# loicland/superpoint_graph

Hardware: AMD Instinct MI355X
Metric: superpoints/sec (embed+ECC fwd+bwd), S3DIS-shaped SPG (higher is better)
Workload: dtype f32; 1 GPU; gru_10_0,f_13 fwd+bwd+Adam; 1 scene/GPU x 1000 sp x 128 pts x 14 f, 5000 edges x 13 f; hipgraph=False, step_call=spg_train_step (one library call: forward + backward), parallelism=single GPU, batchnorm=per-rank statistics, precision=f32

## Files before the change

### include/spg_hip.h

```cpp
#ifndef SPG_HIP_H
#define SPG_HIP_H
#include <stddef.h>
#include <stdint.h>

#ifdef __cplusplus
extern "C" {
#endif

#define SPG_MAX_LAYERS 8
#define SPG_VERSION 200

const char* spg_last_error(void);
int spg_version(void);

size_t spg_graph_workspace_bytes(int N, int n_src, int E);
int spg_graph_build(const int64_t* idxn, const int64_t* degs, int N, int n_src, int E, void* graph_ws, void* stream);
int spg_graph_export(const void* graph_ws, int N, int n_src, int E, int32_t* rowptr, int32_t* src, int32_t* dst,
                     int32_t* rev_rowptr, int32_t* rev_eid, int32_t* hdr, void* stream);

int spg_ecc_aggregate_fwd(int dtype, const void* x, const void* w, const int64_t* idxe, const void* graph_ws, int N,
                          int E, int cin, int cout, int w_is_matrix, void* out, void* stream);
int spg_ecc_aggregate_bwd(int dtype, const void* x, const void* w, const int64_t* idxe, const void* graph_ws, int N,
                          int E, int n_x_rows, int n_w_rows, int cin, int cout, int w_is_matrix, const void* grad_out,
                          void* grad_x, void* grad_w, void* stream);
// ... 246 lines not shown
  float* desc;
  float* grad_desc;
  const spg_eccrnn_cfg* ecc_cfg;
  int E;
  const void* graph_ws;
  const float* edgefeats;
  const void* const* ecc_params;
  void* const* ecc_grads;
  void* ecc_ws; void* ecc_bwd_ws;
  float* ecc_out;
  float* grad_ecc_out;
  int nout, n_classes;
  const float* cls_W; const float* cls_b;
  float* cls_dW; float* cls_db;
  float* cls_work;
  float* logits;
  float* grad_logits;
  const int64_t* target;
  const float* class_weight;
  int64_t ignore_index;
  int reduction_mean;
  float* loss_buf;
  int ptn_slots_clean;
} spg_step_args;
int spg_train_step(const spg_step_args* args, void* stream);
int spg_infer_step(const spg_step_args* args, void* stream);
int spg_cross_entropy_fwd_bwd(const float* logits, const int64_t* target, const float* weight, int N, int C, int64_t ignore_index,
                              int reduction_mean, float* loss, float* lse, float* wsum, float* grad_logits, void* stream);

int spg_ecc_persistent_errors(void);
int spg_ecc_persistent_errors_clear(void);
int spg_ecc_persistent_status(int* errors, int* withheld, int clear);
int spg_prof_read_tag(int tag, double* ms, long* launches, double* flops);

int spg_group_trace(void* buf, int max_launches);
int spg_group_trace_read(int* out, int max);

#define SPG_TILES_VERTICES_PER_BLOCK 32
int spg_neighbourhood_tiles(const float* xyz, const float* rgb, long N, const void* nei, int nei_is_i64, long K, int k, const int64_t* rows,
                            long m, int cloud_rgb, const float* elevation, const float* xyn, int own_rgb, int own_xy, int flags,
                            float* clouds, float* clouds_global, float* diameters, int32_t* error_flag, void* stream);
int spg_augment_whole(const float* xyz, const float* rgb, long N, const float* M, const float* ref_point, const float* noise_xyz,
                      const float* noise_rgb, float* xyz_out, float* rgb_out, void* stream);
size_t spg_random_subgraph_workspace_bytes(long n);
int spg_random_subgraph(const int32_t* rowptr, const uint32_t* inc, const int32_t* ends, long E, long n, int subgraph_size,
                        const int64_t* seeds, int n_seeds, uint8_t* selected_ver, uint8_t* selected_edg, int64_t* state, void* workspace,
                        size_t workspace_bytes, void* stream);
size_t spg_induced_subgraph_workspace_bytes(long n, long E);
int spg_induced_subgraph(const int32_t* ends, long E, long n, const uint8_t* selected_ver, const uint8_t* selected_edg, int64_t* rows,
                         int64_t* new_ver_index, int64_t* kept_edges, int64_t* edg_source, int64_t* edg_target, int64_t* counts,
                         void* workspace, size_t workspace_bytes, void* stream);

enum { SPG_STRUCTURE_IDS_NONE = 0, SPG_STRUCTURE_IDS_OBJECTS = 1, SPG_STRUCTURE_IDS_LABELS = 2, SPG_STRUCTURE_IDS_GIVEN = 3 };
size_t spg_structure_frame_workspace_bytes(long n);
int spg_structure_frame(const float* xyz, long n, float* frame, int32_t* error_flag, void* workspace, size_t workspace_bytes, void* stream);
int spg_structure_vertices(const float* xyz, long n, const float* frame, const uint8_t* rgb_u8, const void* hist, int hist_cols,
                           int id_mode, const void* ids_in, int ids_is_i64, float* elevation, float* xyn, float* rgb, float* geof,
                           int64_t* hard_ids, void* stream);
int spg_structure_edges(const int32_t* knn_idx, long n, int k_local, int k_adj, const int64_t* hard_ids, int64_t* edg_source,
                        int64_t* edg_target, uint8_t* is_transition, uint8_t* active, int32_t* error_flag, void* stream);

size_t spg_plane_workspace_bytes(long n, long n_low, int trials);
int spg_plane_low(const float* xyz, long n, float low_height, int32_t* low_index, int32_t* n_low, int32_t* error_flag, void* workspace,
                  size_t workspace_bytes, void* stream);
int spg_plane_fit(const float* xyz, long n, const int32_t* low_index, long n_low, const int32_t* subsets, int trials, float* elevation,
                  double* coef, double* intercept, float* threshold, uint8_t* inlier_mask, int32_t* result, int32_t* error_flag,
// ... 22 lines not shown
```

### superpoint_graph_amd/_lib.py

```python
from __future__ import annotations

import ctypes
import os
import subprocess

import torch

_HERE = os.path.dirname(os.path.abspath(__file__))
CSRC = os.path.join(_HERE, 'csrc')
LIB_PATH = os.environ.get('SPG_HIP_LIB') or os.path.join(CSRC, 'libspg_hip.so')

SPG_MAX_LAYERS = 8
SPG_MAX_PARTS = 64
c_void_pp = ctypes.POINTER(ctypes.c_void_p)


class PointNetCfg(ctypes.Structure):
    _fields_ = [('nfeat', ctypes.c_int), ('nfeat_stn', ctypes.c_int), ('nfeat_global', ctypes.c_int), ('npts', ctypes.c_int),
                ('n_stn_conv', ctypes.c_int), ('n_stn_fc', ctypes.c_int), ('n_conv', ctypes.c_int), ('n_fc', ctypes.c_int),
                ('stn_conv', ctypes.c_int * SPG_MAX_LAYERS), ('stn_fc', ctypes.c_int * SPG_MAX_LAYERS),
                ('conv', ctypes.c_int * SPG_MAX_LAYERS), ('fc', ctypes.c_int * SPG_MAX_LAYERS),
                ('last_ac', ctypes.c_int), ('bn_eps', ctypes.c_float), ('bn_momentum', ctypes.c_float)]


# ... 144 lines not shown
    'spg_structure_vertices': (_i, [_p, _l, _p, _p, _p, _i, _i, _p, _i, _p, _p, _p, _p, _p, _p]),
    'spg_structure_edges': (_i, [_p, _l, _i, _i, _p, _p, _p, _p, _p, _p, _p]),
    'spg_plane_workspace_bytes': (_sz, [_l, _l, _i]),
    'spg_plane_low': (_i, [_p, _l, ctypes.c_float, _p, _p, _p, _p, _sz, _p]),
    'spg_plane_fit': (_i, [_p, _l, _p, _l, _p, _i, _p, _p, _p, _p, _p, _p, _p, _p, _sz, _p]),
    'spg_parsed_workspace_bytes': (_sz, [_l]),
    'spg_parsed_stats': (_i, [_p, _l, _i, _p, _p, _p, _p, _p, _sz, _p]),
    'spg_parsed_rows': (_i, [_i, _p, _l, _p, _i, _p, _p, _i, _p, _p, _p, _p, _l, _p, _i, _p, _p, _l, _p, _p, _p]),
    'spg_class_count': (_i, [_p, _i, _l, _i, _p, _p]),
    'spg_sample_spg_workspace_bytes': (_sz, [_l, _l]),
    'spg_sample_spg': (_i, [_p, _l, _l, _p, _p, _l, _p, _p, _i, _i, _l, _l, _p, _p, _p, _p, _p, _p, _p, _sz, _p]),
    'spg_edge_features': (_i, [ctypes.POINTER(EdgeFeatureSpecs), _p, _l, _p, _p, _p, _p]),
    'spg_loader_random': (_i, [_p, _p, _p, _i, _i, _i, ctypes.c_uint64, ctypes.c_uint32, _i, ctypes.c_float, _i, ctypes.c_float, _i, _p, _p, _p, _p]),
    'spg_cross_entropy_fwd': (_i, [_p, _p, _p, _i, _i, ctypes.c_int64, _i, _p, _p, _p, _p]),
    'spg_cross_entropy_bwd': (_i, [_p, _p, _p, _p, _p, _p, _i, _i, ctypes.c_int64, _i, _p, _p]),
    'spg_cross_entropy_fwd_bwd': (_i, [_p, _p, _p, _i, _i, ctypes.c_int64, _i, _p, _p, _p, _p, _p]),
    'spg_train_step': (_i, [ctypes.POINTER(StepArgs), _p]),
    'spg_infer_step': (_i, [ctypes.POINTER(StepArgs), _p]),
    'spg_eval_accumulate': (_i, [_p, _i, _l, _i, _i, _p, _p, _p, _p, _p, _p]),
    'spg_set_bn_allreduce': (_i, [_p, _p, _p, _l]),
    'spg_rccl_unique_id': (_i, [_p]),
    'spg_rccl_init': (_i, [_p, _i, _i]),
    'spg_rccl_world_size': (_i, []),
    'spg_rccl_allreduce_sum_f32': (_i, [_p, _l, _p]),
    'spg_rccl_sync_bn': (_i, [_p, _l]),
    'spg_rccl_sync_slots': (_i, [_i]),
    'spg_group_trace': (_i, [_p, _i]),
    'spg_group_trace_read': (_i, [_p, _i]),
    'spg_rccl_allreduce_sum_f64': (_i, [_p, _l, _p]),
    'spg_set_slot_allreduce': (_i, [_p, _p, _i]),
    'spg_rccl_destroy': (_i, []),
    'spg_prof_enable': (None, [_i]),
    'spg_prof_tag': (_i, [_i, _i, _i, _i, _i, _i]),
    'spg_prof_read_tag': (_i, [_i, ctypes.POINTER(ctypes.c_double), ctypes.POINTER(ctypes.c_long), ctypes.POINTER(ctypes.c_double)]),
    'spg_prof_read_shapes': (_i, [ctypes.POINTER(_i), ctypes.POINTER(ctypes.c_double), _i]),
    'spg_tune': (_i, [_i, _i]),
    'spg_prof_read': (_i, [ctypes.POINTER(ctypes.c_double), ctypes.POINTER(ctypes.c_long), ctypes.POINTER(ctypes.c_double), _i]),
}

_lib = None


def build(verbose: bool = False) -> str:
    out = subprocess.run(['make', '-C', CSRC, '-j8'], capture_output=True, text=True)
    if out.returncode != 0:
        raise RuntimeError('building libspg_hip.so failed:\n' + out.stdout[-4000:] + out.stderr[-4000:])
    if verbose:
        print(out.stdout[-2000:])
    return LIB_PATH


def lib():
    global _lib
    if _lib is None:
        if not os.path.exists(LIB_PATH):
            raise RuntimeError(f'{LIB_PATH} not found: the HIP extension is not built '
                               f'(run `python -c "import __graft_entry__ as g; g.build()"` or `make -C {CSRC}`). '
                               'There is no CPU fallback for the product path.')
        L = ctypes.CDLL(LIB_PATH)
        for name, (res, args) in SIGNATURES.items():
            fn = getattr(L, name)
            fn.restype = res
            fn.argtypes = args
        _lib = L
    return _lib

# ... 6 lines not shown
```

### superpoint_graph_amd/csrc/spg_common.h

```cpp
#pragma once
#include <float.h>
#include <hip/hip_runtime.h>
#include <stdint.h>
#include <stdio.h>
#include <string.h>

typedef float f32x16 __attribute__((ext_vector_type(16)));
typedef float f32x4 __attribute__((ext_vector_type(4)));

#define SPG_KC 32
#define SPG_MAX_DEVICES 16
#define SPG_THREADS 256

extern "C" const char* spg_last_error(void);
void spg_set_error(const char* fmt, ...);
enum { SPG_TUNE_NO_PERSIST = 0, SPG_TUNE_DBG = 3, SPG_TUNE_FIN_SLICE_MIN = 4, SPG_TUNE_NO_STAT_ACCUM = 5, SPG_TUNE_NO_HEAD_SERVICE = 6, SPG_TUNE_PRECISION = 7,
       SPG_TUNE_NO_PERSIST_ECC = 8, SPG_TUNE_NO_BN_FOLD = 10, SPG_TUNE_NO_GROUP = 11, SPG_TUNE_NO_BWD_PAIR = 14, SPG_TUNE_NO_ECC_HEAD = 15, SPG_TUNE_NO_NARROW_PAIR = 17, SPG_TUNE_NO_FIRST_CONV_BWD = 18, SPG_TUNE_PX_SPIN_LIMIT = 20, SPG_TUNE_NO_ADAM_GUARD = 21, SPG_TUNE_NO_PAIR_SPLIT = 22, SPG_TUNE_COUNT = 23 };
int spg_tune_get(int key);

#define SPG_CHECK_ARG(cond, msg)                                          \
  do {                                                                    \
    if (!(cond)) {                                                        \
      spg_set_error("%s:%d: bad argument: %s", __FILE__, __LINE__, msg);  \
      return -1;                                                          \
    }                                                                     \
  } while (0)

#define SPG_LAUNCH_CHECK()                                                                  \
  do {                                                                                      \
    hipError_t e__ = hipGetLastError();                                                     \
    if (e__ != hipSuccess) {                                                                \
      spg_set_error("%s:%d: launch failed: %s", __FILE__, __LINE__, hipGetErrorString(e__)); \
      return (int)e__;                                                                      \
    }                                                                                       \
  } while (0)

#define SPG_TRY(expr)           \
  do {                          \
    int rc__ = (expr);          \
    if (rc__ != 0) return rc__; \
  } while (0)

static inline int spg_cdiv(long a, long b) { return (int)((a + b - 1) / b); }

enum {
  SPG_PRO_IDENT = 0,
  SPG_PRO_AFFINE = 1,
  SPG_PRO_CLOUD = 2,
  SPG_PRO_BNBWD = 3,
  SPG_PRO_POOLBWD = 4
// ... 1069 lines not shown
```

### superpoint_graph_amd/csrc/spg_gemm.h

```cpp
#pragma once
#include "spg_common.h"

enum { SPG_EPI_FWD = 0, SPG_EPI_BWD = 1 };

#ifndef SPG_FOLD_SLOTS
#define SPG_FOLD_SLOTS 4
#endif
#define SPG_FOLD_MAX_CONTRIBUTIONS ((long)SPG_FOLD_SLOTS << 17)
inline size_t spg_fold_slot_words(int C) { return (size_t)SPG_FOLD_SLOTS * 4 * C + 8; }
struct SpgBnFold {
  const unsigned long long* slots;
  int C, update_times;
  float momentum, eps;
  double count;
  const float *gamma, *beta;
  float *rm, *rv;
  float *mean, *rstd, *s, *t;
};
struct SpgBnFoldBwd {
  const unsigned long long* slots;
  int C;
  double count;
  const float *s, *mean, *rstd;
  float* consts;
// ... 90 lines not shown

struct SpgProfSpan {
  SpgProfSpan(hipStream_t stream, double flops, int tag, int N, int K);
  ~SpgProfSpan();
  SpgProfSpan(const SpgProfSpan&) = delete;
  SpgProfSpan& operator=(const SpgProfSpan&) = delete;
 private:
  void* impl_;
};

int spg_gemm_ntiles(const SpgGemmParams& p);
inline bool spg_gemm_bwd_stats_want_partials(const SpgGemmParams& g) { return g.w_red && g.N > 64 && g.rows_per_tile > SPG_FC_ROWS && !spg_slot_sync_active(); }
int spg_gemm_row_waves(int rows_per_tile, int N);
int spg_launch_gemm(const SpgGemmParams& p, hipStream_t stream, int* stat_parts = nullptr);

size_t spg_wgrad_workspace_floats(long M, int N, int K);
size_t spg_wgrad_colsum_floats(long M, int N, int K);
int spg_launch_wgrad(SpgWgradParams p, float* dW, float* work, hipStream_t stream);

#define SPG_MAX_REDUCE_JOBS 40
struct SpgReduceJob {
  const float* partial;
  float* out;
  int nsplit, n;
};
struct SpgReduceQueue {
  SpgReduceJob jobs[SPG_MAX_REDUCE_JOBS];
  int njobs = 0;
  float* arena = nullptr;
  size_t arena_floats = 0, used = 0;
};
int spg_queue_wgrad(SpgReduceQueue& q, SpgWgradParams p, float* dW, hipStream_t stream, float* db = nullptr);
bool spg_bwdpair_supported(const SpgGemmParams& g, const SpgOperand& b);
int spg_queue_bwdpair(SpgReduceQueue& q, SpgGemmParams g, const SpgOperand& b, float* dW, hipStream_t stream);
int spg_queue_partials(SpgReduceQueue& q, int nsplit, int n, float* out, float** partial, hipStream_t stream);
int spg_queue_colsum(SpgReduceQueue& q, const float* X, long ld, long M, int N, float* out, hipStream_t stream);
size_t spg_queue_layer_floats(long M, int N, int K);
int spg_flush_reduce(SpgReduceQueue& q, hipStream_t stream);
void spg_reduce_defer(const SpgReduceJob& job);
void spg_reduce_deferred_clear();
int spg_flush_deferred_reduce(hipStream_t stream);
int spg_reduce_ride(SpgReduceQueue& q, hipStream_t stream, size_t max_bytes = (size_t)36 << 20);

size_t spg_bn_finalize_scratch_doubles(int N);
int spg_launch_bn_finalize(const float* stat, const float* stat_cnt, int nparts, long M, int N, const float* gamma,
                           const float* beta, float* running_mean, float* running_var, float momentum, float eps,
                           int update_times, float* mean, float* rstd, float* s, float* t, double* scratch,
                           hipStream_t stream);
bool spg_sync_bn_active();
struct SpgBnEvalJob { int N; const float *gamma, *beta, *rm, *rv; float *s, *t; };
#define SPG_BN_EVAL_MAX_JOBS 40
struct SpgBnEvalBatch { SpgBnEvalJob jobs[SPG_BN_EVAL_MAX_JOBS]; int njobs = 0; };
int spg_launch_bn_eval_batch(const SpgBnEvalBatch& b, float eps, hipStream_t stream);
int spg_launch_bn_eval(int N, const float* gamma, const float* beta, const float* running_mean,
                       const float* running_var, float eps, float* s, float* t, hipStream_t stream);
int spg_launch_bn_bwd_finalize(const float* stat, int ntile, int ldstat, long count, int N, const float* s,
                               const float* mean, const float* rstd, float* consts, float* dgamma, float* dbeta,
                               double* scratch, hipStream_t stream);
int spg_launch_pool_select(const float* pmax, const float* pmin, const int* imax, const int* imin, const float* s,
                           int G, int N, int rows_per_tile, const float* extra, int nextra, float* out, long ldo, int* aidx,
                           hipStream_t stream);
size_t spg_colsum_workspace_floats(int N);
int spg_launch_colsum(const float* X, long ld, long M, int N, float* out, float* work, hipStream_t stream);
int spg_launch_pad_rows(const float* src, long lds, float* dst, long ldd, long rows, int cols, hipStream_t stream);
int spg_launch_stn_dT(const float* clouds, int Ctot, int P, int G, const float* dxy, long ldd, float* dT,
                      hipStream_t stream);

// ... 19 lines not shown
```

### superpoint_graph_amd/csrc/spg_gemm.hip

```cpp
#pragma clang fp contract(off)
#include "../../include/spg_hip.h"
#include "spg_gemm.h"
#include <type_traits>
#include <float.h>
#include <limits.h>
#include <stdarg.h>

static thread_local char g_err[512] = "";
extern "C" const char* spg_last_error(void) { return g_err; }
void spg_set_error(const char* fmt, ...) {
  va_list ap;
  va_start(ap, fmt);
  vsnprintf(g_err, sizeof(g_err), fmt, ap);
  va_end(ap);
}

#include <mutex>
#include <vector>
#ifdef SPG_ATTRIBUTION
#define SPG_DBG(p) ((p).dbg)
#else
#define SPG_DBG(p) 0
#endif
namespace {
struct ProfRec { hipEvent_t a, b; double flops; int tag; int M, N, K; };
bool g_prof_on = false;
std::vector<ProfRec> g_prof;
std::mutex g_prof_mutex;
struct ProfScope {
  hipStream_t st; bool on; ProfRec r;
  ProfScope(hipStream_t s, double flops, int tag = 0, bool enable = true) : st(s), on(g_prof_on && enable) {
    if (on) { (void)hipEventCreate(&r.a); (void)hipEventCreate(&r.b); r.flops = flops; r.tag = tag; r.M = r.N = r.K = 0; (void)hipEventRecord(r.a, st); }
  }
  ~ProfScope() { if (on) { (void)hipEventRecord(r.b, st); std::lock_guard<std::mutex> lock(g_prof_mutex); g_prof.push_back(r); } }
};
}
extern "C" void spg_prof_enable(int on) { g_prof_on = on != 0; }
SpgProfSpan::SpgProfSpan(hipStream_t stream, double flops, int tag, int N, int K) : impl_(nullptr) {
  if (!g_prof_on) return;
  ProfScope* ps = new ProfScope(stream, flops, tag);
  ps->r.N = N; ps->r.K = K;
  impl_ = ps;
}
SpgProfSpan::~SpgProfSpan() { delete static_cast<ProfScope*>(impl_); }

static int g_tune[SPG_TUNE_COUNT] = {0};
static int spg_num_cus() {
  static int n = 0;
  if (n == 0) {
// ... 1945 lines not shown
#pragma unroll
  for (int i = 0; i < TIW; ++i)
#pragma unroll
    for (int q = 0; q < 16; ++q) acc[i][0][q] = 0.f;
  const float xsc = reinterpret_cast<const float*>(kst + 4 * CQ)[wj * 32 + r], xsh = reinterpret_cast<const float*>(kst + 4 * CQ + XQ)[wj * 32 + r];
  __syncthreads();
  int buf = 0;
  SPG_T0();
  for (;;) {
    const int nxt = tile + stride;
    const bool has_next = nxt < ntile;
    const float* dzf = reinterpret_cast<const float*>(smem + buf * BUF4);
    const float* xs = dzf + CQ * SA * 4;
    spg_mfma_chunk_tr_aff<TIW, TIW, IT / 2>(dzf, xs, SA, SX, 0, wi * (32 * TIW) + r, wj * 32 + r, h, xsc, xsh, acc);
    SPG_TP(0);
    __syncthreads();
    SPG_TP(2);
    if (!has_next) break;
    tile = nxt; buf ^= 1;
  }
  SPG_TEND(1);
  __syncthreads();
  float* pb = p.partial + (long)blockIdx.x * CO * CI;
  const int kl = wj * 32 + r;
#pragma unroll
  for (int i = 0; i < TIW; ++i)
#pragma unroll
    for (int q = 0; q < 16; ++q) {
      const int nl = wi * (32 * TIW) + 32 * i + spg_acc_row(q, h);
      __builtin_nontemporal_store(acc[i][0][q], pb + nl * CI + kl);
    }
}

bool spg_bwdpair_supported(const SpgGemmParams& g, const SpgOperand& b) {
  if (g_tune[SPG_TUNE_NO_BWD_PAIR]) return false;
  const int CI = g.N, CO = g.K;
  if (!(g.w_red && g.epi == SPG_EPI_BWD && ((CI == 64 && (CO == 64 || CO == 128)) || (CI == 128 && (CO == 128 || (CO == 256 && !g_tune[SPG_TUNE_NO_PAIR_SPLIT] && g_tune[SPG_TUNE_PRECISION] == 0)))))) return false;
  const int IT = spg_bwdpair_rows(CI);
  if (g.M < IT || g.M % IT != 0) return false;
  const SpgOperand& a = g.a;
  if (a.mode != SPG_PRO_BNBWD && a.mode != SPG_PRO_POOLBWD) return false;
  if (!spg_operand_vec_ok(a) || a.ld < CO) return false;
  if (a.mode == SPG_PRO_POOLBWD && (a.P != 128 || a.ldg < CO)) return false;
  if (CO == 256 && g.fold_bwd.slots != nullptr && g.fold_bwd.C != CO) return false;
  if (b.mode != SPG_PRO_AFFINE || !b.relu || b.c0 == nullptr || b.n_affine != CI || !spg_operand_vec_ok(b) || b.ld < CI) return false;
  if ((g.ldw & 3) != 0 || (((uintptr_t)g.W) & 15) != 0 || g.ldw < CI) return false;
  if (g.Y == nullptr || g.Yp == nullptr || (g.ldy & 3) != 0 || (g.ldyp & 3) != 0 || ((((uintptr_t)g.Y) | ((uintptr_t)g.Yp)) & 15) != 0) return false;
  if (g.Yp != b.X || g.ldyp != b.ld) return false;
  if (g.stat_slots == nullptr || g.mmean == nullptr || g.mrstd == nullptr || g.ms == nullptr || g.mt == nullptr) return false;
  if (g.ms != b.c0 || g.mt != b.c1) return false;
  if (!g.mask_relu || g.n_mask != CI) return false;
  if ((((uintptr_t)g.ms) | ((uintptr_t)g.mt) | ((uintptr_t)g.mmean) | ((uintptr_t)g.mrstd)) & 15) return false;
  const long ntile = g.M / IT;
  const long grid = ntile < spg_num_cus() ? ntile : spg_num_cus();
  return (size_t)grid * CO * CI <= spg_wgrad_workspace_floats(g.M, CO, CI);
}

template <int CO, int CI, int AMODE>
static int launch_bwdpair_t(const SpgBwdPairParams& p, int grid, hipStream_t stream) {
  static bool attr_done = false;
  const size_t lds = spg_bwdpair_lds_bytes<CO, CI>();
  if (!attr_done) {
    hipError_t e = hipFuncSetAttribute(reinterpret_cast<const void*>(&spg_bwdpair_kernel<CO, CI, AMODE>), hipFuncAttributeMaxDynamicSharedMemorySize, (int)lds);
    if (e != hipSuccess) { spg_set_error("hipFuncSetAttribute: %s", hipGetErrorString(e)); return (int)e; }
    attr_done = true;
  }
  hipLaunchKernelGGL((spg_bwdpair_kernel<CO, CI, AMODE>), dim3(grid), dim3(SPG_PAIR_THREADS), lds, stream, p);
  SPG_LAUNCH_CHECK();
  return 0;
}
template <int AMODE>
static int launch_bwdpair_shape(const SpgBwdPairParams& p, int grid, hipStream_t stream) {
  if (p.g.N == 64 && p.g.K == 64) return launch_bwdpair_t<64, 64, AMODE>(p, grid, stream);
  if (p.g.N == 64) return launch_bwdpair_t<128, 64, AMODE>(p, grid, stream);
  return launch_bwdpair_t<128, 128, AMODE>(p, grid, stream);
}

int spg_queue_bwdpair(SpgReduceQueue& q, SpgGemmParams g, const SpgOperand& b, float* dW, hipStream_t stream) {
  SPG_CHECK_ARG(spg_bwdpair_supported(g, b), "shape not supported by the fused backward");
  const int IT = spg_bwdpair_rows(g.N);
  const int ntile = g.M / IT;
  const int grid = ntile < spg_num_cus() ? ntile : spg_num_cus();
  g.ntile = ntile; g.vec_store = 1; g.rows_per_tile = IT;
  const int npass = g.K == 256 ? 2 : 1, COh = g.K / npass;
  for (int h = 0; h < npass; ++h) {
    SpgBwdPairParams p;
    memset(&p, 0, sizeof(p));
    p.g = g; p.b = b;
    p.pass = npass == 1 ? 0 : h + 1;
    if (npass == 2) {
      p.g.K = COh;
      p.g.W = g.W + (long)h * COh * g.ldw;
      p.g.a.X += h * COh; p.g.a.X2 += h * COh;
      if (p.g.a.aidx != nullptr) p.g.a.aidx += h * COh;
      p.g.a.c0 += h * COh; p.g.a.c1 += h * COh; p.g.a.c2 += h * COh; p.g.a.c3 += h * COh;
      if (h == 1) memset(&p.g.fold_bwd, 0, sizeof(p.g.fold_bwd));
    }
    float* dWh = dW + (long)h * COh * g.N;
    if (q.njobs + 1 > SPG_MAX_REDUCE_JOBS) SPG_TRY(spg_flush_reduce(q, stream));
    float* part = dWh;
    if (grid > 1) SPG_TRY(queue_take(q, (size_t)grid * COh * g.N, &part, stream));
    p.partial = part;
    {
      const double flops = 4.0 * (double)g.M * (double)COh * (double)g.N;
      ProfScope prof(stream, flops, SPG_PROF_TAG(4, 64, 64, g.a.mode, SPG_PRO_AFFINE, 1));
      prof.r.M = g.M; prof.r.N = g.N; prof.r.K = COh;
      if (g.a.mode == SPG_PRO_BNBWD) SPG_TRY(launch_bwdpair_shape<SPG_PRO_BNBWD>(p, grid, stream));
      else SPG_TRY(launch_bwdpair_shape<SPG_PRO_POOLBWD>(p, grid, stream));
    }
    if (grid > 1) {
      SpgReduceJob& j = q.jobs[q.njobs++];
      j.partial = part; j.out = dWh; j.nsplit = grid; j.n = COh * g.N;
    }
  }
  SPG_TRY(spg_slot_sync_after(g.stat_slots, spg_fold_slot_words(g.n_mask), stream, false));
  return 0;
}

#define SPG_FIN_SLICES 8

static int* g_fin_counters[SPG_MAX_DEVICES] = {nullptr};
static unsigned g_fin_next[SPG_MAX_DEVICES] = {0};
static std::mutex g_fin_mutex;

static int* spg_fin_counter_window(int n) {
  int dev = 0;
  if (hipGetDevice(&dev) != hipSuccess || dev < 0 || dev >= SPG_MAX_DEVICES) return nullptr;
  std::lock_guard<std::mutex> lock(g_fin_mutex);
  if (g_fin_counters[dev] == nullptr) {
    if (hipMalloc((void**)&g_fin_counters[dev], 4096 * sizeof(int)) != hipSuccess) return nullptr;
    if (hipMemset(g_fin_counters[dev], 0, 4096 * sizeof(int)) != hipSuccess) return nullptr;
  }
  if (g_fin_next[dev] + n > 4096) g_fin_next[dev] = 0;
  int* w = g_fin_counters[dev] + g_fin_next[dev];
  g_fin_next[dev] += n;
  return w;
}

struct SpgBnChannel { float gamma, beta, rm, rv; };
__device__ __forceinline__ SpgBnChannel spg_bn_channel(int c, const float* __restrict__ gamma, const float* __restrict__ beta,
// ... 827 lines not shown
```

### superpoint_graph_amd/csrc/spg_pointnet.hip

```cpp
#include "../../include/spg_hip.h"
#include "spg_ecc.h"
#include "spg_dense.h"
#include "spg_narrow.h"
#include <limits.h>
#include <mutex>
#include <unordered_map>
#include <vector>

namespace {
std::mutex g_gram_mu;
std::unordered_map<const void*, bool> g_gram_filled;
void gram_record(const void* slots, bool filled) { std::lock_guard<std::mutex> lock(g_gram_mu); g_gram_filled[slots] = filled; }
bool gram_recorded(const void* slots) {
  std::lock_guard<std::mutex> lock(g_gram_mu);
  auto it = g_gram_filled.find(slots);
  return it != g_gram_filled.end() && it->second;
}

struct Layer : SpgDenseLayer {
  bool conv = false;
  float* Wpack = nullptr;
  void *Wb_f = nullptr, *Wb_t = nullptr;
};

struct Segment {
  std::vector<int> convs, fcs;
  float* pooled = nullptr;
  long ldpool = 0;
  int* aidx = nullptr;
  int nextra = 0;
  const float* extra = nullptr;
  unsigned long long* gram = nullptr;
};

struct Plan {
  spg_pointnet_cfg cfg;
  int B = 0, P = 0;
  long M = 0;
  bool training = false;
  std::vector<Layer> L;
  Segment stn, main;
  bool has_stn = false;
  float *stat = nullptr, *stat_cnt = nullptr, *pmax = nullptr, *pmin = nullptr;
  double* fin = nullptr;
  int *imax = nullptr, *imin = nullptr;
  unsigned long long* slots_all = nullptr;
  size_t slots_words = 0;
  bool fold = false;
  bool pads_done = false;
  size_t bytes = 0;
// ... 124 lines not shown

SpgDenseBn bn_of(const Plan& pl, int update_times, float* stat, double* fin, float* consts) {
  SpgDenseBn bn;
  bn.training = pl.training; bn.fold = pl.fold; bn.update_times = update_times;
  bn.momentum = pl.cfg.bn_momentum; bn.eps = pl.cfg.bn_eps;
  bn.stat = stat; bn.stat_cnt = pl.stat_cnt; bn.fin = fin; bn.consts = consts;
  return bn;
}

bool fused_eval_convs(Plan& pl, Segment& sg, const float* clouds, const float* stnT, SpgConvStackParams& cp) {
  if (pl.training || sg.convs.size() > SPG_CONVSTACK_MAX_LAYERS) return false;
  memset(&cp, 0, sizeof(cp));
  cp.clouds = clouds; cp.stnT = stnT; cp.B = pl.B; cp.P = pl.P; cp.Ctot = pl.cfg.nfeat; cp.nlayers = (int)sg.convs.size();
  for (size_t k = 0; k < sg.convs.size(); ++k) {
    const Layer& l = pl.L[sg.convs[k]];
    if (!l.bn) return false;
    cp.cin[k] = l.cin; cp.cout[k] = l.cout; cp.W[k] = l.W; cp.bias[k] = l.b; cp.s[k] = l.s; cp.t[k] = l.t;
    cp.Wp[k] = reinterpret_cast<f32x4*>(l.Wpack);
  }
  cp.pmax = pl.pmax; cp.pmin = pl.pmin;
  return spg_conv_stack_eval_supported(cp);
}

int forward_segment(Plan& pl, Segment& sg, const float* clouds, const float* stnT, int update_times, hipStream_t st) {
  SpgConvStackParams cp;
  const bool fused = fused_eval_convs(pl, sg, clouds, stnT, cp);
  if (fused) {
    const Layer& ll = pl.L[sg.convs.back()];
    SPG_TRY(spg_launch_conv_stack_eval(cp, st));
    SPG_TRY(spg_launch_pool_select_parts(pl.pmax, pl.pmin, nullptr, nullptr, ll.s, pl.B, ll.cout, 4, sg.extra, sg.nextra,
                                         sg.pooled, sg.ldpool, nullptr, st));
  }
  size_t kfirst = 0;
  if (pl.training && sg.gram != nullptr) gram_record(sg.gram, false);
  if (!fused && pl.training && pl.fold && sg.gram != nullptr && sg.convs.size() > 2) {
    Layer& l0 = pl.L[sg.convs[0]];
    Layer& l1 = pl.L[sg.convs[1]];
    if (l0.bn && l1.bn && spg_narrow_pair_supported(l0.cin, l0.cout, l1.cout, pl.P, pl.M)) {
      SpgGramParams gp; memset(&gp, 0, sizeof(gp));
      gp.clouds = clouds; gp.stnT = stnT; gp.B = pl.B; gp.P = pl.P; gp.Ctot = pl.cfg.nfeat; gp.nfeat = l0.cin; gp.gram = sg.gram;
      SPG_TRY(spg_launch_cloud_gram(gp, st));
      SPG_TRY(spg_slot_sync_after(sg.gram, spg_gram_slot_words(l0.cin), st, false));
      SpgNarrowPairParams np; memset(&np, 0, sizeof(np));
      np.clouds = clouds; np.stnT = stnT; np.P = pl.P; np.Ctot = pl.cfg.nfeat; np.nfeat = l0.cin; np.nblk = (int)(pl.M / 32);
      np.count = (double)pl.M;
      np.W1 = l0.W; np.b1 = l0.b; np.y1 = l0.y; np.gram = sg.gram; np.gamma1 = l0.gamma; np.beta1 = l0.beta; np.rm1 = l0.rm; np.rv1 = l0.rv;
      np.mean1 = l0.mean; np.rstd1 = l0.rstd; np.s1 = l0.s; np.t1 = l0.t;
      np.update_times = update_times; np.momentum = pl.cfg.bn_momentum; np.eps = pl.cfg.bn_eps;
      np.W2 = l1.W; np.b2 = l1.b; np.y2 = l1.y; np.slots2 = l1.slots;
      SPG_TRY(spg_launch_narrow_pair_fwd(np, st));
      SPG_TRY(spg_slot_sync_after(l1.slots, spg_fold_slot_words(l1.cout), st, false));
      gram_record(sg.gram, true);
      kfirst = 2;
    }
  }
  for (size_t k = kfirst; !fused && k < sg.convs.size(); ++k) {
    Layer& l = pl.L[sg.convs[k]];
    const bool last = k + 1 == sg.convs.size();
    SpgGemmParams g; memset(&g, 0, sizeof(g));
    g.a = input_operand(pl, sg, false, k, clouds, stnT);
    if (k > 0 && pl.fold) g.fold = spg_fold_of(pl.L[sg.convs[k - 1]], pl.M, update_times, pl.cfg.bn_momentum, pl.cfg.bn_eps);
    g.W = l.W; g.ldw = l.cin; g.bias = l.b; g.M = (int)pl.M; g.N = l.cout; g.K = l.cin;
    g.rows_per_tile = pl.P; g.epi = SPG_EPI_FWD; g.Y = l.y; g.ldy = l.ldy;
    if (l.Wb_f != nullptr) { g.Wb = l.Wb_f; g.ldwb = spg_split_ld(l.cin); g.wb_part_bytes = (long)l.cout * g.ldwb * 2; }
    if (last && !pl.training) g.Y = nullptr;
    g.stat = pl.training ? pl.stat : nullptr; g.stat_cnt = pl.stat_cnt;
// ... 86 lines not shown
    d.Yp = first ? sg.pooled : prod.y; d.ldyp = first ? sg.ldpool : prod.ldy;
    d.count = d.stat_rows = first ? pl.M : (long)B;
    d.folds = grp.active();
    SPG_TRY(spg_dense_backward(rq, l, cur, input_operand(pl, sg, true, k, clouds, stnT), B, d, bn_of(pl, 1, s.stat, s.fin, s.consts),
                               pending, &grp, st));
    const int C = prod.cout;
    if (first && s.grad_global != nullptr && sg.nextra > 0)
      SPG_TRY(spg_launch_copy2d(out + C, sg.ldpool, s.grad_global, sg.nextra, B, sg.nextra, st));
    if (!first) {
      cur = spg_op_bnbwd(out, prod.y, prod.ldy, s.consts, C);
    } else {
      memset(&cur, 0, sizeof(cur));
      cur.mode = SPG_PRO_POOLBWD; cur.X = out; cur.ldg = (int)sg.ldpool; cur.aidx = sg.aidx; cur.P = pl.P;
      cur.X2 = prod.y; cur.ld = prod.ldy;
      cur.c0 = s.consts; cur.c1 = s.consts + C; cur.c2 = s.consts + 2 * C; cur.c3 = s.consts + 3 * C;
    }
  }
  }
  float* dz[2] = {s.dzA, s.dzB};
  flip = 0;
  for (int k = (int)sg.convs.size() - 1; k >= 0; --k) {
    Layer& l = pl.L[sg.convs[k]];
    if (k > 0 && pl.fold) {
      Layer& prod = pl.L[sg.convs[k - 1]];
      float* out = dz[flip];
      SpgGemmParams g; memset(&g, 0, sizeof(g));
      g.a = cur; g.W = l.W; g.ldw = l.cin; g.w_red = 1;
      g.M = (int)pl.M; g.N = l.cin; g.K = l.cout; g.rows_per_tile = pl.P;
      g.epi = SPG_EPI_BWD; g.Y = out; g.ldy = l.cin; g.Yp = prod.y; g.ldyp = prod.ldy;
      g.ms = prod.s; g.mt = prod.t; g.mask_relu = 1; g.n_mask = prod.cout;
      g.mmean = prod.mean; g.mrstd = prod.rstd; g.stat_slots = prod.slots_bwd; g.fold_bwd = pending;
      const SpgOperand xin = input_operand(pl, sg, false, k, clouds, stnT);
      if (spg_bwdpair_supported(g, xin)) {
        SPG_TRY(spg_queue_bwdpair(rq, g, xin, l.dW, st));
        if (l.db) SPG_TRY(spg_zero_bytes_async(l.db, sizeof(float) * l.cout, st));
        flip ^= 1;
        pending = spg_fold_bwd_of(prod, pl.M, s.consts);
        cur = spg_op_bnbwd(out, prod.y, prod.ldy, s.consts, prod.cout);
        continue;
      }
    }
    if (k == 0 && pl.fold && sg.gram != nullptr && gram_recorded(sg.gram) && sg.convs.size() > 2 && pending.slots != nullptr && cur.mode == SPG_PRO_BNBWD &&
        cur.ld == l.cout && cur.c0 == s.consts && (!want_dxy || dT_out != nullptr) &&
        spg_narrow_pair_supported(l.cin, l.cout, pl.L[sg.convs[1]].cout, pl.P, pl.M) && spg_first_conv_bwd_supported(l.cin, l.cout, pl.P, pl.M)) {
      SpgFirstConvBwdParams fp; memset(&fp, 0, sizeof(fp));
      fp.clouds = clouds; fp.stnT = stnT; fp.B = pl.B; fp.P = pl.P; fp.Ctot = pl.cfg.nfeat; fp.nfeat = l.cin;
      fp.g = cur.X; fp.W1 = l.W; fp.gram = sg.gram; fp.fold = pending; memset(&pending, 0, sizeof(pending));
      fp.dT = want_dxy ? dT_out : nullptr;
      SPG_TRY(spg_queue_partials(rq, spg_first_conv_bwd_partials(pl.B), l.cout * l.cin, l.dW, &fp.partial, st));
      SPG_TRY(spg_launch_first_conv_bwd(fp, st));
      if (l.db) SPG_TRY(spg_zero_bytes_async(l.db, sizeof(float) * l.cout, st));
      if (want_dxy && dT_done != nullptr) *dT_done = true;
      continue;
    }
    SpgWgradParams w; memset(&w, 0, sizeof(w));
    w.a = cur; w.b = input_operand(pl, sg, false, k, clouds, stnT); w.M = (int)pl.M; w.N = l.cout; w.K = l.cin;
    w.fold = pending; memset(&pending, 0, sizeof(pending));
    w.allow_lowp = 1;
    SPG_TRY(spg_queue_wgrad(rq, w, l.dW, st));
    if (l.db) SPG_TRY(spg_zero_bytes_async(l.db, sizeof(float) * l.cout, st));
    if (k > 0) {
      Layer& prod = pl.L[sg.convs[k - 1]];
      float* out = dz[flip]; flip ^= 1;
      SpgGemmParams g; memset(&g, 0, sizeof(g));
      g.a = cur; g.W = l.W; g.ldw = l.cin; g.w_red = 1;
      g.M = (int)pl.M; g.N = l.cin; g.K = l.cout; g.rows_per_tile = pl.P;
      if (l.Wb_t != nullptr) { g.Wb = l.Wb_t; g.ldwb = spg_split_ld(l.cout); g.wb_part_bytes = (long)l.cin * g.ldwb * 2; }
// ... 160 lines not shown
```

Baseline: 923,100 superpoints/s.

## Add Gram-form fused backward kernel for the pooled last PointNet conv layer

```diff
diff --git a/include/spg_hip.h b/include/spg_hip.h
--- a/include/spg_hip.h
+++ b/include/spg_hip.h
@@ -302,6 +302,7 @@
 int spg_ecc_persistent_errors_clear(void);
 int spg_ecc_persistent_status(int* errors, int* withheld, int clear);
 int spg_prof_read_tag(int tag, double* ms, long* launches, double* flops);
+long spg_poolgram_launches(int reset);
 
 int spg_group_trace(void* buf, int max_launches);
 int spg_group_trace_read(int* out, int max);
diff --git a/superpoint_graph_amd/_lib.py b/superpoint_graph_amd/_lib.py
--- a/superpoint_graph_amd/_lib.py
+++ b/superpoint_graph_amd/_lib.py
@@ -200,6 +200,7 @@
     'spg_rccl_destroy': (_i, []),
     'spg_prof_enable': (None, [_i]),
     'spg_prof_tag': (_i, [_i, _i, _i, _i, _i, _i]),
+    'spg_poolgram_launches': (_l, [_i]),
     'spg_prof_read_tag': (_i, [_i, ctypes.POINTER(ctypes.c_double), ctypes.POINTER(ctypes.c_long), ctypes.POINTER(ctypes.c_double)]),
     'spg_prof_read_shapes': (_i, [ctypes.POINTER(_i), ctypes.POINTER(ctypes.c_double), _i]),
     'spg_tune': (_i, [_i, _i]),
diff --git a/superpoint_graph_amd/csrc/spg_common.h b/superpoint_graph_amd/csrc/spg_common.h
--- a/superpoint_graph_amd/csrc/spg_common.h
+++ b/superpoint_graph_amd/csrc/spg_common.h
@@ -15,7 +15,7 @@
 extern "C" const char* spg_last_error(void);
 void spg_set_error(const char* fmt, ...);
 enum { SPG_TUNE_NO_PERSIST = 0, SPG_TUNE_DBG = 3, SPG_TUNE_FIN_SLICE_MIN = 4, SPG_TUNE_NO_STAT_ACCUM = 5, SPG_TUNE_NO_HEAD_SERVICE = 6, SPG_TUNE_PRECISION = 7,
-       SPG_TUNE_NO_PERSIST_ECC = 8, SPG_TUNE_NO_BN_FOLD = 10, SPG_TUNE_NO_GROUP = 11, SPG_TUNE_NO_BWD_PAIR = 14, SPG_TUNE_NO_ECC_HEAD = 15, SPG_TUNE_NO_NARROW_PAIR = 17, SPG_TUNE_NO_FIRST_CONV_BWD = 18, SPG_TUNE_PX_SPIN_LIMIT = 20, SPG_TUNE_NO_ADAM_GUARD = 21, SPG_TUNE_NO_PAIR_SPLIT = 22, SPG_TUNE_COUNT = 23 };
+       SPG_TUNE_NO_PERSIST_ECC = 8, SPG_TUNE_NO_BN_FOLD = 10, SPG_TUNE_NO_GROUP = 11, SPG_TUNE_NO_BWD_PAIR = 14, SPG_TUNE_NO_ECC_HEAD = 15, SPG_TUNE_NO_NARROW_PAIR = 17, SPG_TUNE_NO_FIRST_CONV_BWD = 18, SPG_TUNE_PX_SPIN_LIMIT = 20, SPG_TUNE_NO_ADAM_GUARD = 21, SPG_TUNE_NO_PAIR_SPLIT = 22, SPG_TUNE_NO_POOL_GRAM = 23, SPG_TUNE_COUNT = 24 };
 int spg_tune_get(int key);
 
 #define SPG_CHECK_ARG(cond, msg)                                          \
diff --git a/superpoint_graph_amd/csrc/spg_gemm.h b/superpoint_graph_amd/csrc/spg_gemm.h
--- a/superpoint_graph_amd/csrc/spg_gemm.h
+++ b/superpoint_graph_amd/csrc/spg_gemm.h
@@ -146,7 +146,8 @@
 };
 int spg_queue_wgrad(SpgReduceQueue& q, SpgWgradParams p, float* dW, hipStream_t stream, float* db = nullptr);
 bool spg_bwdpair_supported(const SpgGemmParams& g, const SpgOperand& b);
-int spg_queue_bwdpair(SpgReduceQueue& q, SpgGemmParams g, const SpgOperand& b, float* dW, hipStream_t stream);
+bool spg_poolgram_shape(const SpgGemmParams& g);
+int spg_queue_bwdpair(SpgReduceQueue& q, SpgGemmParams g, const SpgOperand& b, float* dW, hipStream_t stream, bool gram = false);
 int spg_queue_partials(SpgReduceQueue& q, int nsplit, int n, float* out, float** partial, hipStream_t stream);
 int spg_queue_colsum(SpgReduceQueue& q, const float* X, long ld, long M, int N, float* out, hipStream_t stream);
 size_t spg_queue_layer_floats(long M, int N, int K);
diff --git a/superpoint_graph_amd/csrc/spg_gemm.hip b/superpoint_graph_amd/csrc/spg_gemm.hip
--- a/superpoint_graph_amd/csrc/spg_gemm.hip
+++ b/superpoint_graph_amd/csrc/spg_gemm.hip
@@ -15,6 +15,7 @@
   va_end(ap);
 }
 
+#include <atomic>
 #include <mutex>
 #include <vector>
 #ifdef SPG_ATTRIBUTION
@@ -2026,6 +2027,350 @@
     }
 }
 
+#define SPG_PG_CO 128
+#define SPG_PG_CI 64
+#define SPG_PG_IT 64
+constexpr int SPG_PG_SA = SPG_PG_IT + 1, SPG_PG_SX = SPG_PG_CI + 4, SPG_PG_XQ = SPG_PG_CI / 4;
+constexpr int SPG_PG_BUF4 = SPG_PG_XQ * SPG_PG_SA + 2 * (SPG_PG_IT * SPG_PG_SX / 4) + 2 * SPG_PG_CO / 4;
+constexpr int SPG_PG_KST = 3 * SPG_PG_CO + 3 * SPG_PG_CI;
+constexpr size_t spg_poolgram_lds_bytes() {
+  return (size_t)2 * SPG_PG_BUF4 * 16 + (size_t)(SPG_PG_CO + SPG_PG_CI) * SPG_PG_SX * 4 + (size_t)SPG_PG_KST * 4;
+}
+static_assert(spg_poolgram_lds_bytes() <= 160 * 1024, "LDS of one CU");
+static_assert((SPG_PG_CI * SPG_PG_SX + SPG_PG_CO * SPG_PG_SX + 4 * SPG_PG_CI + 4 * SPG_PG_CI) <= 2 * SPG_PG_BUF4 * 4 && 4 * SPG_PG_CI * SPG_PG_SX + 4 * SPG_PG_CI <= 2 * SPG_PG_BUF4 * 4,
+              "the entry's partials of M and the tail's buffers fit the tile buffers");
+
+__global__ __launch_bounds__(SPG_PAIR_THREADS) void spg_poolgram_kernel(const SpgBwdPairParams p) {
+  constexpr int CO = SPG_PG_CO, CI = SPG_PG_CI, IT = SPG_PG_IT, SA = SPG_PG_SA, SX = SPG_PG_SX, XQ = SPG_PG_XQ, BUF4 = SPG_PG_BUF4;
+  constexpr int NX = IT * XQ / 512, RX = 512 / XQ;
+  constexpr int WJ = 2;
+  constexpr int TPG = 128 / IT;
+  static_assert(NX == 2 && IT == 8 * 8 && CO == 2 * 64, "loader map: 8 waves x 8 rows, two channels per lane");
+  extern __shared__ f32x4 smem[];
+  float* wl = reinterpret_cast<float*>(smem + 2 * BUF4);
+  float* ml = wl + CO * SX;
+  float* kA = ml + CI * SX;
+  float *kD = kA + CO, *kE = kD + CO, *kS = kE + CO, *kT = kS + CI, *kEW = kT + CI;
+  const SpgGemmParams& g = p.g;
+  const int tid = threadIdx.x, lane = tid & 63;
+  const int wave = __builtin_amdgcn_readfirstlane(tid >> 6);
+  const int r = lane & 31, h = lane >> 5;
+  const int role = wave >> 2;
+  const int wi = (wave & 3) / WJ, wj = (wave & 3) % WJ;
+  const int ntile = g.ntile, stride = (int)gridDim.x;
+  int tile = (int)blockIdx.x;
+  auto buf_a = [&](int b) __attribute__((always_inline)) { return smem + b * BUF4; };
+  auto buf_x = [&](int b) __attribute__((always_inline)) { return reinterpret_cast<float*>(smem + b * BUF4 + XQ * SA); };
+  auto buf_sp = [&](int b) __attribute__((always_inline)) { return reinterpret_cast<float*>(smem + b * BUF4 + XQ * SA) + IT * SX; };
+  auto buf_row = [&](int b) __attribute__((always_inline)) { return reinterpret_cast<int*>(reinterpret_cast<float*>(smem + b * BUF4 + XQ * SA) + 2 * IT * SX); };
+  auto buf_cf = [&](int b) __attribute__((always_inline)) { return reinterpret_cast<float*>(smem + b * BUF4 + XQ * SA) + 2 * IT * SX + CO; };
+  float* gl = reinterpret_cast<float*>(smem);
+  float* ssl = gl + CI * SX;
+  float* sgl = ssl + CO * SX;
+  float* xch = sgl + 4 * CI;
+
+  auto prologue = [&](auto wload) __attribute__((always_inline)) {
+    constexpr bool WLOAD = decltype(wload)::value;
+    constexpr int NWQ = CO * XQ / 512;
+    f32x4 wq[NWQ];
+    if constexpr (WLOAD) {
+#pragma unroll
+      for (int k = 0; k < NWQ; ++k) {
+        const int i = tid + k * 512, co = i / XQ, q = i % XQ;
+        wq[k] = *reinterpret_cast<const f32x4*>(g.W + (long)co * g.ldw + 4 * q);
+      }
+    }
+    if (blockIdx.x == 0 && tid == 0) spg_slots_count_add(g.stat_slots, g.n_mask, g.stat_rows != 0 ? g.stat_rows : (long)g.M);
+    if (g.fold_bwd.slots != nullptr) spg_bn_fold_bwd(g.fold_bwd, blockIdx.x == 0);
+    if (tid < CO) {
+      const float A = g.a.c0[tid], B = g.a.c1[tid], C = g.a.c2[tid], D = g.a.c3[tid];
+      const float bias = g.bias != nullptr ? g.bias[tid] : 0.f;
+      kA[tid] = A; kD[tid] = D;
+      kE[tid] = fmaf(A, B, (bias - C) * D);
+    }
+    if (tid < CI) { kS[tid] = p.b.c0[tid]; kT[tid] = p.b.c1[tid]; }
+    if constexpr (WLOAD) {
+#pragma unroll
+      for (int k = 0; k < NWQ; ++k) {
+        const int i = tid + k * 512, co = i / XQ, q = i % XQ;
+        *reinterpret_cast<f32x4*>(wl + co * SX + 4 * q) = wq[k];
+      }
+    }
+    __syncthreads();
+    {
+      const int ib = (wave & 3) >> 1, jb = wave & 1, cb = 32 * (wave >> 2);
+      f32x16 macc;
+#pragma unroll
+      for (int q = 0; q < 16; ++q) macc[q] = 0.f;
+#pragma unroll
+      for (int kk = 0; kk < 16; ++kk) {
+        const int c = cb + 2 * kk + h;
+        macc = __builtin_amdgcn_mfma_f32_32x32x2f32(wl[c * SX + ib * 32 + r] * kD[c], wl[c * SX + jb * 32 + r], macc, 0, 0, 0);
+      }
+      float* scr = reinterpret_cast<float*>(smem) + (wave >> 2) * CI * SX;
+#pragma unroll
+      for (int q = 0; q < 16; ++q) scr[(ib * 32 + spg_acc_row(q, h)) * SX + jb * 32 + r] = macc[q];
+      if (tid >= SPG_PAIR_THREADS - 4 * CI) {
+        const int part = (tid - (SPG_PAIR_THREADS - 4 * CI)) >> 6;
+        float ew = 0.f;
+#pragma unroll 16
+        for (int c = 32 * part; c < 32 * part + 32; ++c) ew = fmaf(kE[c], wl[c * SX + lane], ew);
+        reinterpret_cast<float*>(smem)[4 * CI * SX + part * CI + lane] = ew;
+      }
+    }
+    __syncthreads();
+    {
+      const int o = (tid >> 4) * SX + 4 * (tid & 15);
+      const float* scr = reinterpret_cast<const float*>(smem);
+      const f32x4 p0 = *reinterpret_cast<const f32x4*>(scr + o), p1 = *reinterpret_cast<const f32x4*>(scr + CI * SX + o);
+      const f32x4 p2 = *reinterpret_cast<const f32x4*>(scr + 2 * CI * SX + o), p3 = *reinterpret_cast<const f32x4*>(scr + 3 * CI * SX + o);
+      *reinterpret_cast<f32x4*>(ml + o) = -(((p0 + p1) + p2) + p3);
+      if (tid < CI) {
+        const float* q = scr + 4 * CI * SX + tid;
+        kEW[tid] = ((q[0] + q[CI]) + q[2 * CI]) + q[3 * CI];
+      }
+    }
+    __syncthreads();
+  };
+
+  auto tail = [&]() __attribute__((always_inline)) {
+    if (wave >= 8) return;
+    const int cb = 32 * (wave >> 1), jb = 32 * (wave & 1);
+    f32x16 t;
+#pragma unroll
+    for (int q = 0; q < 16; ++q) t[q] = 0.f;
+#pragma unroll
+    for (int kk = 0; kk < CI / 2; ++kk) {
+      const int k = 2 * kk + h;
+      t = __builtin_amdgcn_mfma_f32_32x32x2f32(wl[(cb + r) * SX + k], gl[k * SX + jb + r], t, 0, 0, 0);
+    }
+    const int j = jb + r;
+    const float sj = ((sgl[j] + sgl[CI + j]) + sgl[2 * CI + j]) + sgl[3 * CI + j];
+    float* pb = p.partial + (long)blockIdx.x * CO * CI + j;
+#pragma unroll
+    for (int q = 0; q < 16; ++q) {
+      const int c = cb + spg_acc_row(q, h);
+      __builtin_nontemporal_store(fmaf(-kD[c], t[q], fmaf(-kE[c], sj, ssl[c * SX + j])), pb + c * CI);
+    }
+  };
+
+  if (role >= 2) {
+    const int lt = tid - 512, lw = wave - 8;
+    const int xq = lt % XQ, rx = lt / XQ;
+    const unsigned ox = ((unsigned)rx * (unsigned)p.b.ld + 4u * (unsigned)xq) * 4u, sx = (unsigned)RX * (unsigned)p.b.ld * 4u;
+    struct Regs {
+      f32x4 px[NX];
+      int ai[2];
+      float pg[2];
+    };
+    Regs R0, R1;
+    auto load_tile = [&](Regs& R, int t) __attribute__((always_inline)) {
+      const float* xb = p.b.X + (long)t * IT * p.b.ld;
+#pragma unroll
+      for (int i = 0; i < NX; ++i) R.px[i] = spg_ld16(xb, ox + sx * i);
+      const long go = (long)(t / TPG) * g.a.ldg;
+      R.ai[0] = g.a.aidx[go + lane]; R.ai[1] = g.a.aidx[go + 64 + lane];
+      R.pg[0] = g.a.X[go + lane]; R.pg[1] = g.a.X[go + 64 + lane];
+    };
+    auto store_tile = [&](const Regs& R, int t, int buf) __attribute__((always_inline)) {
+      f32x4* a4 = buf_a(buf);
+      float* xs = buf_x(buf);
+      const f32x4 ks = *reinterpret_cast<const f32x4*>(kS + 4 * xq), kt = *reinterpret_cast<const f32x4*>(kT + 4 * xq);
+#pragma unroll
+      for (int i = 0; i < NX; ++i) {
+        const int row = rx + RX * i;
+        *reinterpret_cast<f32x4*>(xs + row * SX + 4 * xq) = R.px[i];
+        f32x4 av;
+#pragma unroll
+        for (int e = 0; e < 4; ++e) av[e] = fmaxf(fmaf(R.px[i][e], ks[e], kt[e]), 0.f);
+        a4[xq * SA + row] = av;
+      }
+      const int prow = (t % TPG) * IT, lo = 8 * lw;
+      const int row0 = R.ai[0] - prow, row1 = R.ai[1] - prow;
+      const float cf0 = kA[lane] * R.pg[0], cf1 = kA[64 + lane] * R.pg[1];
+      if (lw == 0) {
+        buf_row(buf)[lane] = row0; buf_row(buf)[64 + lane] = row1;
+        buf_cf(buf)[lane] = cf0; buf_cf(buf)[64 + lane] = cf1;
+      }
+      float* sp = buf_sp(buf);
+#pragma unroll
+      for (int u = 0; u < 8; ++u) sp[(lo + u) * SX + lane] = 0.f;
+      auto hits = [&](int rowv, float cfv, int cbase) __attribute__((always_inline)) {
+        unsigned long long m = __ballot(rowv >= lo && rowv < lo + 8);
+        while (m != 0ull) {
+          const int cl = __builtin_amdgcn_readfirstlane(__builtin_ctzll(m));
+          m &= m - 1ull;
+          const int rr = __builtin_amdgcn_readlane(rowv, cl);
+          const float cf = __int_as_float(__builtin_amdgcn_readlane(__float_as_int(cfv), cl));
+          float* d = sp + rr * SX + lane;
+          *d = fmaf(cf, wl[(cbase + cl) * SX + lane], *d);
+        }
+      };
+      hits(row0, cf0, 0);
+      hits(row1, cf1, 64);
+    };
+    load_tile(R0, tile);
+    if (tile + stride < ntile) load_tile(R1, tile + stride);
+    prologue(std::false_type{});
+    store_tile(R0, tile, 0);
+    if (tile + 2 * stride < ntile) load_tile(R0, tile + 2 * stride);
+    __syncthreads();
+    for (;;) {
+      int nxt = tile + stride;
+      bool has_next = nxt < ntile;
+      if (has_next) {
+        store_tile(R1, nxt, 1);
+        if (nxt + 2 * stride < ntile) load_tile(R1, nxt + 2 * stride);
+      }
+      __syncthreads();
+      if (!has_next) break;
+      tile = nxt;
+      nxt = tile + stride;
+      has_next = nxt < ntile;
+      if (has_next) {
+        store_tile(R0, nxt, 0);
+        if (nxt + 2 * stride < ntile) load_tile(R0, nxt + 2 * stride);
+      }
+      __syncthreads();
+      if (!has_next) break;
+      tile = nxt;
+    }
+    __syncthreads();
+    tail();
+    return;
+  }
+
+  prologue(std::true_type{});
+  if (role == 0) {
+    constexpr int CW = 32, LD = SX, LPR = CW / 4, RPI = 64 / LPR;
+    const int colw = wj * CW, roww = wi * 32;
+    const int lr = lane / LPR, lc = 4 * (lane % LPR);
+    const int col = colw + lc;
+    const f32x4 sc = *reinterpret_cast<const f32x4*>(g.ms + col), sh = *reinterpret_cast<const f32x4*>(g.mt + col);
+    const f32x4 mean = *reinterpret_cast<const f32x4*>(g.mmean + col), rstd = *reinterpret_cast<const f32x4*>(g.mrstd + col);
+    const unsigned oo0 = (unsigned)lr * (unsigned)g.ldy + (unsigned)lc;
+    const float init = -kEW[colw + r];
+    f32x4 s1 = {0.f, 0.f, 0.f, 0.f}, s2 = s1;
+    __syncthreads();
+    int buf = 0;
+    for (;;) {
+      const int nxt = tile + stride;
+      const bool has_next = nxt < ntile;
+      f32x16 acc;
+#pragma unroll
+      for (int q = 0; q < 16; ++q) acc[q] = init;
+      spg_mfma_tile_or<CI / 8, 2>(buf_a(buf), ml, SA, SX, roww + r, colw + r, h, acc);
+      float* st = buf_sp(buf) + roww * LD + colw;
+      const float* yl = buf_x(buf) + (roww + lr) * SX + col;
+      float* yo = g.Y + ((long)tile * IT + roww) * g.ldy + colw;
+#pragma unroll
+      for (int q = 0; q < 16; ++q) st[spg_acc_row(q, h) * LD + r] += acc[q];
+#pragma unroll
+      for (int u = 0; u < 32 / RPI; ++u) {
+        f32x4 v = *reinterpret_cast<const f32x4*>(st + (lr + RPI * u) * LD + lc);
+        const f32x4 yv = *reinterpret_cast<const f32x4*>(yl + RPI * u * SX);
+        const f32x4 act = spg_fma4(yv, sc, sh), xhat = (yv - mean) * rstd;
+#pragma unroll
+        for (int e = 0; e < 4; ++e)
+          if (!(act[e] > 0.f)) v[e] = 0.f;
+        s1 += v;
+        s2 = spg_fma4(v, xhat, s2);
+        __builtin_nontemporal_store(v, reinterpret_cast<f32x4*>(yo + oo0 + (unsigned)(RPI * u) * (unsigned)g.ldy));
+      }
+      __syncthreads();
+      if (!has_next) break;
+      tile = nxt; buf ^= 1;
+    }
+    const int cl = colw + lc;
+#pragma unroll
+    for (int off = LPR; off < 64; off <<= 1) {
+#pragma unroll
+      for (int e = 0; e < 4; ++e) { s1[e] += __shfl_xor(s1[e], off, 64); s2[e] += __shfl_xor(s2[e], off, 64); }
+    }
+    if (wi != 0 && lane < LPR) {
+      *reinterpret_cast<f32x4*>(xch + (wi * CI + cl) * 2) = s1;
+      *reinterpret_cast<f32x4*>(xch + (wi * CI + cl) * 2 + 4) = s2;
+    }
+    __syncthreads();
+    if (wi == 0 && lane < LPR) {
+      s1 += *reinterpret_cast<const f32x4*>(xch + (1 * CI + cl) * 2);
+      s2 += *reinterpret_cast<const f32x4*>(xch + (1 * CI + cl) * 2 + 4);
+#pragma unroll
+      for (int e = 0; e < 4; ++e) spg_slots_add(g.stat_slots, g.n_mask, cl + e, (double)s1[e], (double)s2[e]);
+    }
+    tail();
+    return;
+  }
+
+  f32x16 acc[1][1];
+#pragma unroll
+  for (int q = 0; q < 16; ++q) acc[0][0][q] = 0.f;
+  const float xsc = kS[wj * 32 + r], xsh = kT[wj * 32 + r];
+  const int wt = tid - 256;
+  const int sc_c = wt >> 1, sc_q = 8 * (wt & 1);
+  const int sg_j = wt & 63, sg_r = 16 * (wt >> 6);
+  f32x4 ss[8];
+#pragma unroll
+  for (int u = 0; u < 8; ++u) ss[u] = f32x4{0.f, 0.f, 0.f, 0.f};
+  float sg = 0.f;
+  __syncthreads();
+  int buf = 0;
+  for (;;) {
+    const int nxt = tile + stride;
+    const bool has_next = nxt < ntile;
+    const float* af = reinterpret_cast<const float*>(buf_a(buf));
+    spg_mfma_chunk_tr_aff<1, 1, IT / 2>(af, buf_x(buf), SA, SX, 0, wi * 32 + r, wj * 32 + r, h, xsc, xsh, acc);
+    const int row = buf_row(buf)[sc_c];
+    if (row >= 0 && row < IT) {
+      const float cf = buf_cf(buf)[sc_c];
+      const f32x4* a4 = buf_a(buf);
+#pragma unroll
+      for (int u = 0; u < 8; ++u) {
+        const f32x4 av = a4[(sc_q + u) * SA + row];
+#pragma unroll
+        for (int e = 0; e < 4; ++e) ss[u][e] = fmaf(cf, av[e], ss[u][e]);
+      }
+    }
+    {
+      const float* ac = af + ((sg_j >> 2) * SA + sg_r) * 4 + (sg_j & 3);
+#pragma unroll
+      for (int u = 0; u < 16; ++u) sg += ac[4 * u];
+    }
+    __syncthreads();
+    if (!has_next) break;
+    tile = nxt; buf ^= 1;
+  }
+#pragma unroll
+  for (int q = 0; q < 16; ++q) gl[(wi * 32 + spg_acc_row(q, h)) * SX + wj * 32 + r] = acc[0][0][q];
+#pragma unroll
+  for (int u = 0; u < 8; ++u) *reinterpret_cast<f32x4*>(ssl + sc_c * SX + 4 * (sc_q + u)) = ss[u];
+  sgl[(wt >> 6) * CI + sg_j] = sg;
+  __syncthreads();
+  tail();
+}
+
+bool spg_poolgram_shape(const SpgGemmParams& g) {
+  return g.a.mode == SPG_PRO_POOLBWD && g.N == SPG_PG_CI && g.K == SPG_PG_CO && g.a.P == 128 && g.a.aidx != nullptr &&
+         (((uintptr_t)g.W) & 15) == 0 && (g.ldw & 3) == 0;
+}
+
+static std::atomic<long> g_poolgram_launches{0};
+extern "C" long spg_poolgram_launches(int reset) { return reset ? g_poolgram_launches.exchange(0) : g_poolgram_launches.load(); }
+
+static int launch_poolgram(const SpgBwdPairParams& p, int grid, hipStream_t stream) {
+  static bool attr_done = false;
+  const size_t lds = spg_poolgram_lds_bytes();
+  if (!attr_done) {
+    hipError_t e = hipFuncSetAttribute(reinterpret_cast<const void*>(&spg_poolgram_kernel), hipFuncAttributeMaxDynamicSharedMemorySize, (int)lds);
+    if (e != hipSuccess) { spg_set_error("hipFuncSetAttribute: %s", hipGetErrorString(e)); return (int)e; }
+    attr_done = true;
+  }
+  hipLaunchKernelGGL(spg_poolgram_kernel, dim3(grid), dim3(SPG_PAIR_THREADS), lds, stream, p);
+  SPG_LAUNCH_CHECK();
+  g_poolgram_launches.fetch_add(1);
+  return 0;
+}
+
 bool spg_bwdpair_supported(const SpgGemmParams& g, const SpgOperand& b) {
   if (g_tune[SPG_TUNE_NO_BWD_PAIR]) return false;
   const int CI = g.N, CO = g.K;
@@ -2070,8 +2415,9 @@
   return launch_bwdpair_t<128, 128, AMODE>(p, grid, stream);
 }
 
-int spg_queue_bwdpair(SpgReduceQueue& q, SpgGemmParams g, const SpgOperand& b, float* dW, hipStream_t stream) {
+int spg_queue_bwdpair(SpgReduceQueue& q, SpgGemmParams g, const SpgOperand& b, float* dW, hipStream_t stream, bool gram) {
   SPG_CHECK_ARG(spg_bwdpair_supported(g, b), "shape not supported by the fused backward");
+  SPG_CHECK_ARG(!gram || spg_poolgram_shape(g), "shape not supported by the Gram form of the pooled layer");
   const int IT = spg_bwdpair_rows(g.N);
   const int ntile = g.M / IT;
   const int grid = ntile < spg_num_cus() ? ntile : spg_num_cus();
@@ -2096,10 +2442,12 @@
     if (grid > 1) SPG_TRY(queue_take(q, (size_t)grid * COh * g.N, &part, stream));
     p.partial = part;
     {
-      const double flops = 4.0 * (double)g.M * (double)COh * (double)g.N;
+      const double flops = gram ? 4.0 * (double)g.M * (double)g.N * (double)g.N + 2.0 * (double)grid * COh * (double)g.N * (double)g.N
+                                : 4.0 * (double)g.M * (double)COh * (double)g.N;
       ProfScope prof(stream, flops, SPG_PROF_TAG(4, 64, 64, g.a.mode, SPG_PRO_AFFINE, 1));
       prof.r.M = g.M; prof.r.N = g.N; prof.r.K = COh;
-      if (g.a.mode == SPG_PRO_BNBWD) SPG_TRY(launch_bwdpair_shape<SPG_PRO_BNBWD>(p, grid, stream));
+      if (gram) SPG_TRY(launch_poolgram(p, grid, stream));
+      else if (g.a.mode == SPG_PRO_BNBWD) SPG_TRY(launch_bwdpair_shape<SPG_PRO_BNBWD>(p, grid, stream));
       else SPG_TRY(launch_bwdpair_shape<SPG_PRO_POOLBWD>(p, grid, stream));
     }
     if (grid > 1) {
diff --git a/superpoint_graph_amd/csrc/spg_pointnet.hip b/superpoint_graph_amd/csrc/spg_pointnet.hip
--- a/superpoint_graph_amd/csrc/spg_pointnet.hip
+++ b/superpoint_graph_amd/csrc/spg_pointnet.hip
@@ -16,6 +16,9 @@
   auto it = g_gram_filled.find(slots);
   return it != g_gram_filled.end() && it->second;
 }
+
+void poolgram_record(const void* aidx, bool gram) { gram_record(aidx, gram); }
+bool poolgram_recorded(const void* aidx) { return gram_recorded(aidx); }
 
 struct Layer : SpgDenseLayer {
   bool conv = false;
@@ -206,6 +209,11 @@
                                          sg.pooled, sg.ldpool, nullptr, st));
   }
   size_t kfirst = 0;
+  if (pl.training) {
+    const Layer& lp = pl.L[sg.convs.back()];
+    poolgram_record(sg.aidx, pl.fold && sg.convs.size() > 1 && lp.cin == 64 && lp.cout == 128 && pl.P == 128 && lp.bn &&
+                                 spg_gemm_precision() == 0 && !spg_tune_get(SPG_TUNE_NO_BWD_PAIR) && !spg_tune_get(SPG_TUNE_NO_POOL_GRAM));
+  }
   if (pl.training && sg.gram != nullptr) gram_record(sg.gram, false);
   if (!fused && pl.training && pl.fold && sg.gram != nullptr && sg.convs.size() > 2) {
     Layer& l0 = pl.L[sg.convs[0]];
@@ -358,7 +366,9 @@
       g.mmean = prod.mean; g.mrstd = prod.rstd; g.stat_slots = prod.slots_bwd; g.fold_bwd = pending;
       const SpgOperand xin = input_operand(pl, sg, false, k, clouds, stnT);
       if (spg_bwdpair_supported(g, xin)) {
-        SPG_TRY(spg_queue_bwdpair(rq, g, xin, l.dW, st));
+        const bool gram = k + 1 == (int)sg.convs.size() && poolgram_recorded(sg.aidx) && spg_poolgram_shape(g);
+        if (gram) g.bias = l.b;
+        SPG_TRY(spg_queue_bwdpair(rq, g, xin, l.dW, st, gram));
         if (l.db) SPG_TRY(spg_zero_bytes_async(l.db, sizeof(float) * l.cout, st));
         flip ^= 1;
         pending = spg_fold_bwd_of(prod, pl.M, s.consts);
```

Result: no change. 931,700 superpoints/s, median of 6 (+0.9%).
